# kgnlp/allophant

Measured on AMD Instinct MI355X. Metric: encoder frames/sec (whole node), 10s x 32 utterances @16kHz, higher is better.
Workload: dtype f16x3

## Files before the change

### __graft_entry__.py

```python
import os
import subprocess
import sys

ROOT = os.path.dirname(os.path.abspath(__file__))
if ROOT not in sys.path:
    sys.path.insert(0, ROOT)


def build() -> None:
    jobs = str(min(8, os.cpu_count() or 1))
    subprocess.check_call(["make", "-C", os.path.join(ROOT, "allophant_amd", "csrc"), "-j", jobs])
    out_dir = os.path.join(ROOT, "oracle", "_build")
    os.makedirs(out_dir, exist_ok=True)
    subprocess.check_call(["gcc", "-O2", "-shared", "-fPIC", "-o", os.path.join(out_dir, "liboracle_int.so"),
                           os.path.join(ROOT, "oracle", "oracle_int.c")])
    import allophant_amd
    from allophant_amd import lib

    handle = lib.load()
    missing = [s for s in lib.EXPORTS + lib.ALLOPHONE_EXPORTS + lib.BEAM_EXPORTS + lib.RESAMPLE_EXPORTS + lib.EDIT_EXPORTS + lib.EDIT_WEIGHTED_EXPORTS
               + lib.ALIGN_EXPORTS + lib.SCORE_EXPORTS + lib.SEARCH_EXPORTS + lib.RESTRICT_EXPORTS + lib.LONG_EXPORTS
               if not hasattr(handle, s)]
    if missing:
        raise RuntimeError(f"liballophant_amx.so lacks exported symbols: {missing}")


# ... 45 lines not shown
```

### allophant_amd/csrc/amx_api.hip

```cpp
#include "../../include/allophant_amx.h"
#include "../../include/allophant_amx_allophones.h"
#include "../../include/allophant_amx_beam.h"
#include "../../include/allophant_amx_align.h"
#include "../../include/allophant_amx_score.h"
#include "../../include/allophant_amx_search.h"
#include "../../include/allophant_amx_restrict.h"
#include "../../include/allophant_amx_long.h"
#include "../../include/allophant_amx_resample.h"
#include "../../include/allophant_amx_edit.h"
#include "amx_common.h"

#include <algorithm>
#include <cmath>
#include <cstdio>
#include <cstring>
#include <initializer_list>
#include <map>
#include <cstdlib>
#include <string>
#include <vector>

using namespace amx;

namespace {
// ... 117 lines not shown
    struct GraphEntry {
        std::vector<int64_t> key;
        hipGraphExec_t exec = nullptr;
        hipGraph_t graph = nullptr;
        uint64_t last_use = 0;
        hipStream_t last_stream = nullptr;
    };
    static constexpr int GRAPH_CAP = 32;
    std::vector<GraphEntry> graphs;
    std::vector<std::vector<int64_t>> graph_seen;
    static constexpr int GRAPH_SEEN = 8;
    hipStream_t capture_stream = nullptr;
    bool graph_broken = false;
    uint64_t ws_gen = 0, graph_clock = 0;
    int64_t graph_captures = 0, graph_replays = 0;
    struct RangeSlot {
        int* host = nullptr;
        hipEvent_t ev = nullptr;
        bool pending = false, cont = false;
        uint64_t pass_id = 0;
    };
    static constexpr int RANGE_SLOTS = 8;
    RangeSlot range[RANGE_SLOTS];
    int range_next = 0;
    int64_t range_carry = 0;
    std::string range_carry_ids;
    uint64_t pass_counter = 0;
    int range_chain_seen = 0;
    bool range_chain_open = false;
    int last_N = 0;
// ... 1063 lines not shown
    HIPCHK(h, hipStreamSynchronize(s));
    for (int i = 0; i < amx_handle_s::PIN_SLOTS; ++i) {
        if (h->h_lengths_pinned[i]) {
            (void)hipHostFree(h->h_lengths_pinned[i]);
            (void)hipHostFree(h->h_frames_pinned[i]);
            (void)hipHostFree(h->h_rowoff_pinned[i]);
        }
        HIPCHK(h, hipHostMalloc((void**)&h->h_lengths_pinned[i], (size_t)N * 8));
        HIPCHK(h, hipHostMalloc((void**)&h->h_frames_pinned[i], (size_t)N * 4));
        HIPCHK(h, hipHostMalloc((void**)&h->h_rowoff_pinned[i], (size_t)(3 * N + 1) * 4));
        if (!h->pin_event[i]) HIPCHK(h, hipEventCreateWithFlags(&h->pin_event[i], hipEventDisableTiming));
        h->pin_busy[i] = false;
    }
    h->pinned_cap = N;
    return AMX_OK;
}

static int plan_conv_tiles(amx_handle h, PassPlan& P, int slot, const std::vector<int>& valid_rows, hipStream_t s) {
    const amx_config& c = h->cfg;
    const int N = P.N;
    size_t total_tiles = 0;
    constexpr int64_t TR = GEMM_LN_TILE_ROWS;
    for (int i = 1; i < c.n_conv; ++i) total_tiles += (size_t)((N * P.Ts[i + 1] + TR - 1) / TR);
    if (h->tiles_cap[slot] < total_tiles) {
        if (h->h_tiles_pinned[slot]) (void)hipHostFree(h->h_tiles_pinned[slot]);
        h->h_tiles_pinned[slot] = nullptr;
        h->tiles_cap[slot] = 0;
        HIPCHK(h, hipHostMalloc((void**)&h->h_tiles_pinned[slot], (total_tiles + total_tiles / 4 + 64) * 4));
        h->tiles_cap[slot] = total_tiles + total_tiles / 4 + 64;
    }
// ... 211 lines not shown
        P.frames_host.assign(pin_frames, pin_frames + N);
    }
    P.stream_in_planes = NT == 2;
    if (P.stable && c.layers > 0 && D % 64 == 0 && D <= 2048) {
        WS("ln_rowps", (size_t)P.Mrows * 16, P.ln_rowps);
        WS("ln_coef", (size_t)P.Mrows * 8, P.ln_coef);
        WS("ln_partial", (size_t)P.Mrows * (D / 64) * 8, P.ln_partial);
        const Layer& ly = h->layers[0];
        const int prec = P.prec;
        P.fold = gemm_ln_fold_ok(prec, P.as_consumer(P.qkv_params(h, ly), ly.c_qkv)) &&
                 gemm_ln_fold_ok(prec, P.as_producer(P.oproj_params(h, ly), false)) &&
                 gemm_ln_fold_ok(prec, P.as_consumer(P.ffn1_params(h, ly), ly.c_1)) &&
                 gemm_ln_fold_ok(prec, P.as_producer(P.ffn2_params(h, ly), false)) &&
                 gemm_ln_fold_ok(prec, P.as_producer(P.ffn2_params(h, ly), true));
    }
    ++h->pass_counter;
    h->last_fold = P.fold;
    h->last_packed = P.packed_early ? 2 : (P.packed ? 1 : 0);
    h->last_attention = c.layers > 0 ? attention_form(P.attn_params()) : -1;
    h->last_rows = P.Mrows;
    h->last_graph = 0;
#undef WS
    return AMX_OK;
}

static int enqueue_pass(amx_handle h, const PassPlan& P, hipStream_t s) {
    const amx_config& c = h->cfg;
    const int prec = P.prec, N = P.N, C = P.C, D = P.D, T = P.T;
    const int64_t M = P.M, Mh = P.Mh;
    void* hbuf = P.hbuf;
    bool refused = false;
    auto gemm = [&](const GemmParams& g, int cls = -1) {
        Timed t_(h, cls < 0 ? gemm_class(prec, g) : cls);
        refused |= !launch_gemm(prec, P.with_ws(g), s);
    };
    if (P.needs_qkv_zero) {
        launch_zero(P.qb, P.qkv_bytes, s);
        launch_zero(P.kb, P.qkv_bytes, s);
        launch_zero(P.vtb, P.qkv_bytes, s);
    }
    if (P.packed) {
        const size_t row_b = (size_t)P.dhp * 2, tail = (size_t)(P.TpTot - P.Mp) * row_b, pitch = (size_t)P.TpTot * row_b;
        for (void* buf : {P.qb, P.kb, P.vtb})
            launch_zero_2d((char*)buf + (size_t)P.Mp * row_b, pitch, tail, (size_t)P.NT * P.H, s);
    }
    if (!(P.flags & AMX_FLAG_CONTINUE)) launch_zero(h->nonfinite, 4, s);
    { Timed t_(h, AMX_KC_OTHER); launch_audio_stats(P.d_audio, (const int64_t*)P.d_len, N, P.L, (double*)P.d_partial, (float*)P.d_stats, c.do_normalize, s); }
    if (h->gn) {
        Timed t_(h, AMX_KC_CONV0);
// ... 1243 lines not shown
```

### allophant_amd/csrc/amx_common.h

```cpp
#pragma once
#include <hip/hip_runtime.h>
#include <stdint.h>
#include <string>
#include <type_traits>

struct amx_resample_geometry;
struct amx_resample_row;
struct amx_long_window;
struct amx_long_block;

namespace amx {

typedef _Float16 f16;
typedef __bf16 bf16;
typedef __attribute__((ext_vector_type(8))) _Float16 f16x8;
typedef __attribute__((ext_vector_type(8))) __bf16 bf16x8;
typedef __attribute__((ext_vector_type(4))) _Float16 f16x4;
typedef __attribute__((ext_vector_type(4))) __bf16 bf16x4;
typedef __attribute__((ext_vector_type(2))) _Float16 f16x2;
typedef __attribute__((ext_vector_type(2))) __bf16 bf16x2;
typedef __attribute__((ext_vector_type(2))) float f32x2;
typedef __attribute__((ext_vector_type(4))) float f32x4;
typedef __attribute__((ext_vector_type(16))) float f32x16;

// ... 202 lines not shown
    float* splitk_ws;
    int64_t splitk_ws_elems;
    int splits;
    int64_t split_out;
    const int* tile_list;
    int n_tiles;
    int defer_fixup;
    int a_taps;
    int64_t a_tap_stride;
    unsigned long long* stamps;
    const float4* ln_rowps;
    float2* ln_partial;
    int ln_res_planes;
    const float2* row_coef;
    const float* col_c;
};

extern bool g_force_generic_gemm;
bool launch_gemm(int prec, const GemmParams& p, hipStream_t stream);
bool gemm_uses_pp(int prec, const GemmParams& p);
bool gemm_fuses_ln(int prec, const GemmParams& p);
int gemm_ln_tap_minor_slice(int prec, const GemmParams& p);
int gemm_planned_splits(int prec, const GemmParams& p);
bool fixup_rownorm_eligible(const GemmParams& p);
void launch_fixup_rownorm(int prec, const GemmParams& p, int splits, const float* gamma, const float* beta, float eps, void* out_p,
                          int64_t out_plane, int64_t ldp, float* out_ln, int64_t ldo_ln, hipStream_t stream);
bool gemm_ln_fold_ok(int prec, const GemmParams& p);
void launch_gemm_grouped(int prec, const GemmParams& p, int groups, hipStream_t stream);

struct AttnParams {
    const void* q;
    const void* k;
    const void* v;
    int64_t qk_plane;
    void* out;
    int64_t out_plane;
    const int* frame_len;
    int N, H, T, Tp, dh;
// ... 231 lines not shown
```

### allophant_amd/csrc/amx_gemm.hip

```cpp
#include "amx_common.h"
#include <algorithm>
#include <cstdlib>
#include <type_traits>

namespace amx {

bool g_force_generic_gemm = false;

namespace {

#include "amx_gemm_tile.inc"
#include "amx_gemm_pp.inc"
#include "amx_gemm_ln.inc"

int device_cus() {
    static int per_device[MAX_DEVICES] = {};
    const int dev = current_device();
    int& cus = per_device[dev];
    if (!cus) {
        hipDeviceProp_t prop;
        if (hipGetDeviceProperties(&prop, dev) == hipSuccess) cus = prop.multiProcessorCount;
        if (cus <= 0) cus = 256;
        cus -= cus % 8;
        if (cus < 8) cus = 8;
// ... 125 lines not shown
    q.zbias = q.zoutp = 0;
    return q;
}

template <typename T, int NT, int MI, int NI, int FOLD>
void launch_pp_tiles(const GemmParams& p, int splits, hipStream_t stream) {
    static OncePerDevice attr;
    constexpr int lds = pp::lds_bytes(NT, MI, NI);
    if (attr.first())
        (void)hipFuncSetAttribute((const void*)gemm_pp_kernel<T, NT, MI, NI, FOLD>, hipFuncAttributeMaxDynamicSharedMemorySize, lds);
    if (FOLD) splits = 1;
    const int tiles = ((p.N + NI * 64 - 1) / (NI * 64)) * ((p.M + MI * 32 - 1) / (MI * 32));
    const int cus = device_cus();
    const int units = tiles * splits;
    dim3 grid(units < cus ? units : cus, 1, 1);
    if (splits > 1) {
        hipLaunchKernelGGL((gemm_pp_kernel<T, NT, MI, NI, FOLD>), grid, dim3(512), lds, stream, split_view(p, splits));
        if (!p.defer_fixup) launch_fixup<T, NT>(p, splits, stream);
    } else {
        hipLaunchKernelGGL((gemm_pp_kernel<T, NT, MI, NI, FOLD>), grid, dim3(512), lds, stream, p);
    }
}

void pp_plan(int NT, const GemmParams& p, int* mi_out, int* splits_out, int* ni_out) {
    const int cus = device_cus();
    const double loop = (double)p.K * (NT > 1 ? 3 : 1);
    double best = 1e30;
    *mi_out = 8;
    *splits_out = 1;
    *ni_out = 4;
    for (int mi = 8; mi >= 4; mi -= 4)
        for (int ni = 4; ni >= 3; --ni) {
            const int tiles = ((p.N + ni * 64 - 1) / (ni * 64)) * ((p.M + mi * 32 - 1) / (mi * 32));
            const double per_unit = (480.0 + 60.0 * mi) * (ni == 4 ? 1.0 : 1.1);
            const double unit_loop = loop * mi / 8.0 * (ni == 4 ? 1.0 : 0.75 * 1.06);
            int64_t smax = 1;
// ... 209 lines not shown
    if (p.ln_partial) {
        if (r.ni != 4 || p.N % 64 || p.N > 2048 || !p.out_p || !p.ln_rowps || p.act || p.mode || p.row_len || p.row_coef) return false;
        if (p.ln_res_planes ? NT != 2 : (!p.out_f32 || !p.residual)) return false;
        if (NT == 2 && (p.out_plane != PLANE_IL || p.ldp % 32)) return false;
        if (p.ldp % 8 || ((uintptr_t)p.out_p & 15) || ((uintptr_t)p.ln_partial & 7) || ((uintptr_t)p.ln_rowps & 15)) return false;
    }
    if (p.row_coef) {
        if (!p.col_c || ((uintptr_t)p.col_c & 15) || ((uintptr_t)p.row_coef & 7) || p.residual || p.row_len) return false;
        if (p.mode != 1 && (!p.out_p || p.out_f32)) return false;
    }
    return true;
}

int gemm_planned_splits(int prec, const GemmParams& p) { return route_of(prec, p).splits; }

bool fixup_rownorm_eligible(const GemmParams& p) {
    return p.splitk_ws && p.out_f32 && !p.out_p && p.act == 0 && p.mode == 0 && !p.row_len && !p.ln_gamma && p.N % 4 == 0 &&
           p.N <= 1024 && p.ldo % 4 == 0 && (!p.residual || p.ldr % 4 == 0) && !((uintptr_t)p.out_f32 & 15) &&
           !((uintptr_t)p.residual & 15) && !((uintptr_t)p.bias & 15) && p.zout == 0;
}

void launch_fixup_rownorm(int prec, const GemmParams& p, int splits, const float* gamma, const float* beta, float eps, void* out_p,
                          int64_t out_plane, int64_t ldp, float* out_ln, int64_t ldo_ln, hipStream_t stream) {
    AMX_DISPATCH(prec, (launch_fixup_rownorm_t<T16, NT>(p, splits, gamma, beta, eps, out_p, out_plane, ldp, out_ln, ldo_ln, stream)));
}

bool launch_gemm(int prec, const GemmParams& p_in, hipStream_t stream) {
    const GemmParams p = with_vec_flag(p_in);
    const GemmRoute r = gemm_route(prec_planes(prec), p);
    if (!r.launches) return false;
// ... 11 lines not shown
```

### allophant_amd/csrc/amx_gemm_ln.inc

```

namespace ppw {
constexpr int BM = 128, BN = 512, KS = 32;
static_assert(BM == GEMM_LN_TILE_ROWS, "amx_forward builds the tile lists of ragged batches for this tile height");
constexpr int A_BYTES = BM * 64, W_BYTES = BN * 64, SLOT = A_BYTES + W_BYTES, W_OFF = A_BYTES;
constexpr int LDS_BYTES = 4 * SLOT;
constexpr int EPI_BASE = 2 * SLOT;
constexpr int RED_BASE = EPI_BASE + 8 * pp::EPI_WAVE;
constexpr int AJ = 1, WJ = 4;
}

template <typename T, int NT>
__global__ __launch_bounds__(512, 2) void gemm_ln_kernel(const GemmParams p) {
    typedef typename Vec8<T>::type V8;
    typedef __attribute__((address_space(3))) void* lds_ptr_t;
    extern __shared__ __attribute__((aligned(16))) unsigned char smem[];

    const int tid = threadIdx.x;
    int lane = tid & 63;
    const int wave = __builtin_amdgcn_readfirstlane(tid >> 6);
    const int grp = wave >> 2, wc = wave & 3;
    const int total = p.tile_list ? p.n_tiles : (p.M + ppw::BM - 1) / ppw::BM;

    const int rd_chunk = ((lane >> 4) ^ ((lane >> 2) & 2)) << 4;
    const int a_rd = (grp * 64 + (lane & 15)) * 64 + rd_chunk;
// ... 292 lines not shown
    const int w_rd = ppi::A_BYTES + (grp * 256 + wc * 64 + (lane & 15)) * 128 + rd_chunk;

    const __amdgpu_buffer_rsrc_t w_rsrc = __builtin_amdgcn_make_buffer_rsrc((void*)p.W, 0, -1, 0x00020000);
    uint32_t w_off[2], a_off[4];
#pragma unroll
    for (int par = 0; par < 2; ++par) {
        const int row = (grp * 32 + wc * 8 + par) * 8 + (lane >> 3);
        const int lc = (lane & 7) ^ ((row >> 1) & 7);
        w_off[par] = (uint32_t)((EM * (int64_t)row * p.ldw + lc * 8) * 2);
    }
    const uint32_t w_step = (uint32_t)(p.ldw * 32 * EM);
    int m0 = 0;
    __amdgpu_buffer_rsrc_t a_rsrc;
    auto setup_tile = [&](int i) {
        m0 = (p.tile_list ? p.tile_list[i] : i) * ppi::BM;
        const int64_t b0 = m0 / p.rows_per_batch;
        const int64_t a_tile = b0 * p.a_batch_stride + (m0 - b0 * p.rows_per_batch) * p.lda;
        a_rsrc = __builtin_amdgcn_make_buffer_rsrc((void*)((const T*)p.A + EM * a_tile), 0, -1, 0x00020000);
#pragma unroll
        for (int j = 0; j < 4; ++j) {
            const int row = (wc * 4 + j) * 8 + ((tid & 63) >> 3);
            const int lc = (tid & 7) ^ ((row >> 1) & 7);
            int rr = m0 + row;
            rr = rr < p.M ? rr : p.M - 1;
            const int64_t b = rr / p.rows_per_batch;
            const int64_t t = rr - b * p.rows_per_batch;
            a_off[j] = (uint32_t)((EM * (b * p.a_batch_stride + t * p.lda - a_tile) + lc * 8) * 2);
        }
    };
    const int taps = p.a_taps > 1 ? p.a_taps : 1;
    const uint32_t tap_bytes = (uint32_t)(p.a_tap_stride * EM * 2);
    auto dma_slice = [&](int slot, int slice) {
        unsigned char* base = smem + slot * ppi::SLICE;
        const uint32_t so = (uint32_t)slice * 128;
        if (grp == 0) {
            uint32_t so_a = so;
            if (taps > 1) {
                const uint32_t cs = (uint32_t)slice / (uint32_t)taps, pos = (uint32_t)slice - cs * (uint32_t)taps;
                const uint32_t tap = pos ? (uint32_t)taps - pos : 0u;
                so_a = tap * tap_bytes + cs * 128;
            }
#pragma unroll
// ... 28 lines not shown
#pragma unroll
        for (int prod = 0; prod < NT + 1; ++prod) {
            const int pw = NT == 2 ? (prod == 1 ? 1 : 0) : prod, pa = NT == 2 ? (prod == 2 ? 1 : 0) : prod;
#pragma unroll
            for (int ni = 0; ni < 4; ++ni)
#pragma unroll
                for (int mi = 0; mi < MI; ++mi) mfma16_acc(acc[ni][mi], fw[pw][ni], fa[pa][mi]);
        }
        __builtin_amdgcn_s_setprio(0);
        asm volatile("s_waitcnt vmcnt(0)" ::: "memory");
        __builtin_amdgcn_sched_barrier(0);
        __builtin_amdgcn_s_barrier();
        __builtin_amdgcn_sched_barrier(0);
    };

    int it = blockIdx.x;
    setup_tile(it);
    dma_slice(0, 0);
    for (;;) {
#pragma unroll
        for (int i = 0; i < 4; ++i)
#pragma unroll
            for (int j = 0; j < MI; ++j) acc[i][j] = f32x4{0.f, 0.f, 0.f, 0.f};
        const int nk = p.K / KSL;
        asm volatile("s_waitcnt vmcnt(0)" ::: "memory");
        __builtin_amdgcn_s_barrier();
        if (grp == 1) __builtin_amdgcn_s_barrier();
        for (int k = 0; k < nk; k += 2) {
            phase(std::integral_constant<int, 0>{}, k, nk);
            phase(std::integral_constant<int, 1>{}, k + 1, nk);
        }
        if (grp == 0) __builtin_amdgcn_s_barrier();
        asm volatile("s_nop 15\n\ts_nop 15" ::: "memory");

        const int mw = m0, nw = grp * 256 + wc * 64;
        const int next = it + gridDim.x;
        const bool has_next = next < total;
        if (has_next) {
            setup_tile(next);
            dma_slice(0, 0);
        }

        asm volatile("" : "+v"(lane));
        {
            const int lr = lane & 15, lg = lane >> 4;
            const float scale = p.scale;
            float* red = (float*)(smem + ppi::RED_BASE);
#pragma unroll
            for (int ni = 0; ni < 4; ++ni) {
                const float4 b4 = p.bias ? *(const float4*)(p.bias + nw + ni * 16 + 4 * lg) : make_float4(0.f, 0.f, 0.f, 0.f);
#pragma unroll
                for (int mi = 0; mi < MI; ++mi) {
                    acc[ni][mi][0] = fmaf(acc[ni][mi][0], scale, b4.x);
                    acc[ni][mi][1] = fmaf(acc[ni][mi][1], scale, b4.y);
                    acc[ni][mi][2] = fmaf(acc[ni][mi][2], scale, b4.z);
                    acc[ni][mi][3] = fmaf(acc[ni][mi][3], scale, b4.w);
// ... 43 lines not shown
                for (int mi = 0; mi < MI; ++mi) {
                    const f32x2 g01 = gelu_fast2(f32x2{fmaf((acc[ni][mi][0] - mean[mi]) * rstd[mi], g4.x, e4.x),
                                                       fmaf((acc[ni][mi][1] - mean[mi]) * rstd[mi], g4.y, e4.y)});
                    const f32x2 g23 = gelu_fast2(f32x2{fmaf((acc[ni][mi][2] - mean[mi]) * rstd[mi], g4.z, e4.z),
                                                       fmaf((acc[ni][mi][3] - mean[mi]) * rstd[mi], g4.w, e4.w)});
                    acc[ni][mi][0] = g01[0];
                    acc[ni][mi][1] = g01[1];
                    acc[ni][mi][2] = g23[0];
                    acc[ni][mi][3] = g23[1];
                }
            }
            float* es = (float*)(smem + ppi::EPI_BASE + wave * pp::EPI_WAVE);
            if (mw + ppi::BM <= p.M) pp_epilogue_p16<T, NT, false, false, MI, true>(p, acc, es, lane, mw, nw);
            else pp_epilogue_generic<T, NT, MI, true>(p, acc, es, lane, mw, nw, nullptr);
        }
        if (!has_next) break;
        it = next;
        lgkm_wait0();
        __builtin_amdgcn_s_barrier();
    }
}
```

### allophant_amd/csrc/amx_gemm_pp.inc

```

namespace pp {
constexpr int BN = 256;
constexpr int EPI_WAVE = 32 * 64 * 4;
template <int MI, int NI = 4>
struct Ring {
    static constexpr int A_BYTES = MI * 32 * 128, W_BYTES = NI * 64 * 128, SLICE = A_BYTES + W_BYTES;
    static constexpr int NSL = MI == 8 ? 2 : 3, DIST = NSL - 1;
    static constexpr int EPI_BASE = DIST * SLICE;
    static constexpr int LDS_BYTES = (NSL * SLICE > EPI_BASE + 8 * EPI_WAVE) ? NSL * SLICE : EPI_BASE + 8 * EPI_WAVE;
};
constexpr int lds_bytes(int NT, int MI, int NI = 4) {
    return MI == 8 ? (NI == 4 ? Ring<8, 4>::LDS_BYTES : Ring<8, 3>::LDS_BYTES) : (NI == 4 ? Ring<4, 4>::LDS_BYTES : Ring<4, 3>::LDS_BYTES);
}
constexpr int epi_base(int NT, int MI, int NI = 4) {
    return MI == 8 ? (NI == 4 ? Ring<8, 4>::EPI_BASE : Ring<8, 3>::EPI_BASE) : (NI == 4 ? Ring<4, 4>::EPI_BASE : Ring<4, 3>::EPI_BASE);
}
__device__ __forceinline__ int es_idx(int row, int chunk) { return row * 64 + ((chunk ^ (row & 7)) << 2); }
}

__device__ __forceinline__ void mfma16_acc(f32x4& c, f16x8 a, f16x8 b) {
    asm volatile("v_mfma_f32_16x16x32_f16 %0, %1, %2, %0" : "+v"(c) : "v"(a), "v"(b));
}
__device__ __forceinline__ void mfma16_acc(f32x4& c, bf16x8 a, bf16x8 b) {
    asm volatile("v_mfma_f32_16x16x32_bf16 %0, %1, %2, %0" : "+v"(c) : "v"(a), "v"(b));
// ... 204 lines not shown
    for (int q = 0; q < MI / 2; ++q) {
        float2 cf[4];
        if (COEF) {
#pragma unroll
            for (int i = 0; i < 4; ++i) cf[i] = cf_all[q][i];
        }
        pp_stage_round(es, acc, q, lane);
        f32x4 c[4][2];
#pragma unroll
        for (int i = 0; i < 4; ++i) {
            c[i][0] = *(const f32x4*)(es + pp::es_idx(i * 8 + rs, 2 * c8));
            c[i][1] = *(const f32x4*)(es + pp::es_idx(i * 8 + rs, 2 * c8 + 1));
        }
#pragma unroll
        for (int i = 0; i < 4; ++i) {
            float v[8];
            if (COEF) {
                const float as = cf[i].x * scale, bs = cf[i].y;
                v[0] = fmaf(c[i][0][0], as, fmaf(bs, cc0.x, b0.x)); v[1] = fmaf(c[i][0][1], as, fmaf(bs, cc0.y, b0.y));
                v[2] = fmaf(c[i][0][2], as, fmaf(bs, cc0.z, b0.z)); v[3] = fmaf(c[i][0][3], as, fmaf(bs, cc0.w, b0.w));
                v[4] = fmaf(c[i][1][0], as, fmaf(bs, cc1.x, b1.x)); v[5] = fmaf(c[i][1][1], as, fmaf(bs, cc1.y, b1.y));
                v[6] = fmaf(c[i][1][2], as, fmaf(bs, cc1.z, b1.z)); v[7] = fmaf(c[i][1][3], as, fmaf(bs, cc1.w, b1.w));
            } else {
                v[0] = fmaf(c[i][0][0], scale, b0.x); v[1] = fmaf(c[i][0][1], scale, b0.y); v[2] = fmaf(c[i][0][2], scale, b0.z);
                v[3] = fmaf(c[i][0][3], scale, b0.w); v[4] = fmaf(c[i][1][0], scale, b1.x); v[5] = fmaf(c[i][1][1], scale, b1.y);
                v[6] = fmaf(c[i][1][2], scale, b1.z); v[7] = fmaf(c[i][1][3], scale, b1.w);
            }
            union { typename Vec2<T>::type h[4]; V8 v; } hv, lv;
#pragma unroll
            for (int r = 0; r < 4; ++r) {
                f32x2 x = {v[2 * r], v[2 * r + 1]};
                if (ACT) x = gelu_fast2(x);
                lv.h[r] = typename Vec2<T>::type{(T)0.f, (T)0.f};
                split16x2<T, NT>(x, hv.h[r], lv.h[r]);
            }
            T* dst;
            if (QK) {
                dst = base + ((int64_t)b * p.H * p.Tp + t) * row_stride;
                t += 8;
                const bool wrap = t >= p.T;
                t -= wrap ? p.T : 0;
                b += wrap ? 1 : 0;
            } else {
                dst = base + (int64_t)(q * 32 + i * 8) * row_stride;
            }
            *(V8*)dst = hv.v;
// ... 137 lines not shown
    int lane = tid & 63;
    const int wave = __builtin_amdgcn_readfirstlane(tid >> 6);
    const int grp = wave >> 2, wc = wave & 3;
    const int ntn = (p.N + BNK - 1) / BNK, ntm = (p.M + BMK - 1) / BMK;
    const int tiles = ntn * ntm;
    const int total = tiles * p.splits;

    const int rd_chunk = ((lane >> 4) ^ ((lane >> 1) & 7)) << 4;
    const int a_rd = (grp * HALF + (lane & 15)) * 128 + rd_chunk;
    const int w_rd = R::A_BYTES + (wc * (16 * NI) + (lane & 15)) * 128 + rd_chunk;

    int m0 = 0, n0 = 0, ks = 0;
    __amdgpu_buffer_rsrc_t a_rsrc, w_rsrc;
    uint32_t a_off[4], w_off[2];
    const uint32_t w_step = (uint32_t)(p.ldw * 32 * EM);
    auto setup_tile = [&](int unit) {
        ks = unit / tiles;
        const int i = unit - ks * tiles;
        const int total = tiles;
        const int xcd = i & 7, q = total >> 3, r = total & 7;
        const int j = (xcd < r ? xcd * (q + 1) : r * (q + 1) + (xcd - r) * q) + (i >> 3);
        constexpr int GM = 8;
        const int per_group = GM * ntn;
        const int group = j / per_group;
        const int first_m = group * GM;
        const int gsize = ntm - first_m < GM ? ntm - first_m : GM;
        const int in_group = j - group * per_group;
        m0 = (first_m + in_group % gsize) * BMK;
        n0 = (in_group / gsize) * BNK;
        const int m0c = m0 < p.M ? m0 : p.M - 1, n0c = n0 < p.N ? n0 : p.N - 1;
        const int64_t b0 = m0c / p.rows_per_batch;
        const int64_t a_tile = b0 * p.a_batch_stride + (m0c - b0 * p.rows_per_batch) * p.lda;
        const int64_t k_first = (int64_t)ks * p.K;
        a_rsrc = __builtin_amdgcn_make_buffer_rsrc((void*)((const T*)p.A + EM * (a_tile + k_first)), 0, -1, 0x00020000);
        const int64_t w_bytes = ((int64_t)(p.N - n0c) * p.ldw - k_first) * 2 * EM;
        w_rsrc = __builtin_amdgcn_make_buffer_rsrc((void*)((const T*)p.W + EM * ((int64_t)n0c * p.ldw + k_first)), 0,
                                                   (int)(uint32_t)(w_bytes < 0xFFFFFFFFll ? w_bytes : 0xFFFFFFFFll), 0x00020000);
#pragma unroll
        for (int jj = 0; jj < APW2; ++jj) {
            const int row = (grp * (2 * MI) + wc * APW2 + jj) * 8 + ((tid & 63) >> 3);
            const int lc = (tid & 7) ^ ((row >> 1) & 7);
            int rr = m0 + row;
            rr = rr < p.M ? rr : p.M - 1;
            const int64_t b = rr / p.rows_per_batch;
            const int64_t t = rr - b * p.rows_per_batch;
            a_off[jj] = (uint32_t)((EM * (b * p.a_batch_stride + t * p.lda - a_tile) + lc * 8) * 2);
        }
#pragma unroll
        for (int par = 0; par < 2; ++par) {
            const int row = (wc * WPW + par) * 8 + ((tid & 63) >> 3);
            const int lc = (tid & 7) ^ ((row >> 1) & 7);
            w_off[par] = (uint32_t)((EM * (int64_t)row * p.ldw + lc * 8) * 2);
        }
    };

    f32x4 acc[NI][MI];
    V8 fa[2][MI], fw[2][NI];

    auto dma_slice = [&](int slot, int slice) {
#ifdef AMX_ABLATE_NO_DMA
        return;
#endif
        unsigned char* base = smem + slot * R::SLICE;
        const uint32_t so = (uint32_t)slice * 128;
#pragma unroll
        for (int j = 0; j < APW2; ++j)
            __builtin_amdgcn_raw_ptr_buffer_load_lds(a_rsrc, (lds_ptr_t)(base + (grp * (2 * MI) + wc * APW2 + j) * 1024), 16, a_off[j], so,
// ... 16 lines not shown
            case 1: asm volatile("s_waitcnt vmcnt(1)" ::: "memory"); break;
            case 2: asm volatile("s_waitcnt vmcnt(2)" ::: "memory"); break;
            case 3: asm volatile("s_waitcnt vmcnt(3)" ::: "memory"); break;
            case 4: asm volatile("s_waitcnt vmcnt(4)" ::: "memory"); break;
            case 5: asm volatile("s_waitcnt vmcnt(5)" ::: "memory"); break;
            case 6: asm volatile("s_waitcnt vmcnt(6)" ::: "memory"); break;
            case 7: asm volatile("s_waitcnt vmcnt(7)" ::: "memory"); break;
            case 8: asm volatile("s_waitcnt vmcnt(8)" ::: "memory"); break;
            case 9: asm volatile("s_waitcnt vmcnt(9)" ::: "memory"); break;
            case 10: asm volatile("s_waitcnt vmcnt(10)" ::: "memory"); break;
            case 11: asm volatile("s_waitcnt vmcnt(11)" ::: "memory"); break;
            default: asm volatile("s_waitcnt vmcnt(12)" ::: "memory"); break;
        }
    };
#ifdef AMX_PP_STAMP
    unsigned long long st_load = 0, st_bar1 = 0, st_mfma = 0, st_vm = 0, st_bar2 = 0, st_prev = 0, st_begin_rt = 0, st_loop = 0;
    auto stamp = []() -> unsigned long long {
        unsigned long long t;
        __builtin_amdgcn_sched_barrier(0);
        asm volatile("s_memtime %0\n\ts_waitcnt lgkmcnt(0)" : "=s"(t)::"memory");
        __builtin_amdgcn_sched_barrier(0);
        return t;
    };
    {
        unsigned long long t;
        asm volatile("s_memrealtime %0\n\ts_waitcnt lgkmcnt(0)" : "=s"(t)::"memory");
        st_begin_rt = t;
    }
    const unsigned long long st_begin = stamp();
#endif
    auto phase = [&](auto slot_c, int k, int nk) {
// ... 45 lines not shown
        const unsigned long long t3 = stamp();
        st_mfma += t3 - t2;
#endif
        if (R::DIST == 2 && k + 2 < nk) wait_dma(grp == 0 ? CNT_A + CNT_W : CNT_A);
        else asm volatile("s_waitcnt vmcnt(0)" ::: "memory");
#ifdef AMX_PP_STAMP
        const unsigned long long t4 = stamp();
        st_vm += t4 - t3;
        st_prev = t4;
#endif
        __builtin_amdgcn_sched_barrier(0);
        __builtin_amdgcn_s_barrier();
        __builtin_amdgcn_sched_barrier(0);
    };
    int it = blockIdx.x;
    setup_tile(it);
    stage_head();
    for (;;) {
#pragma unroll
        for (int i = 0; i < NI; ++i)
#pragma unroll
            for (int j = 0; j < MI; ++j) acc[i][j] = f32x4{0.f, 0.f, 0.f, 0.f};
#ifdef AMX_PP_STAMP
        const unsigned long long st_l0 = stamp();
        st_prev = 0;
#endif
        {
            const int nk = p.K / KSL;
            if (R::DIST == 2) wait_dma(grp == 0 ? APW2 + WPW : APW2);
            else asm volatile("s_waitcnt vmcnt(0)" ::: "memory");
            __builtin_amdgcn_s_barrier();
// ... 2 lines not shown
                for (int k = 0; k < nk; k += 2) {
                    phase(std::integral_constant<int, 0>{}, k, nk);
                    phase(std::integral_constant<int, 1>{}, k + 1, nk);
                }
            } else {
                for (int k = 0;;) {
                    phase(std::integral_constant<int, 0>{}, k, nk);
                    if (++k == nk) break;
                    phase(std::integral_constant<int, 1>{}, k, nk);
                    if (++k == nk) break;
                    phase(std::integral_constant<int, 2>{}, k, nk);
                    if (++k == nk) break;
                }
            }
        }
        if (grp == 0) __builtin_amdgcn_s_barrier();
        asm volatile("s_nop 15\n\ts_nop 15" ::: "memory");
#ifdef AMX_PP_STAMP
        st_loop += stamp() - st_l0;
#endif

        const int mw = m0 + grp * HALF, nw = n0 + wc * (16 * NI);
        float* out_f32 = p.out_f32 ? p.out_f32 + (int64_t)ks * p.split_out : nullptr;
        const int next = it + gridDim.x;
        const bool has_next = next < total;
        if (has_next) {
            setup_tile(next);
            stage_head();
        }

#ifndef AMX_ABLATE_NO_EPI
        asm volatile("" : "+v"(lane));
        if (nw < p.N && mw < p.M) {
            float* es = (float*)(smem + pp::epi_base(NT, MI, NI) + wave * pp::EPI_WAVE);
            bool done = false;
            if constexpr (FOLD == 1) {
                if (mw + HALF <= p.M && nw + 16 * NI <= p.N && p.vec_ok) {
                    if (p.mode == 1) {
                        if (p.T >= 8 && p.dh % 8 == 0 && p.qk_plane % 8 == 0 && !(((uintptr_t)p.q | (uintptr_t)p.k | (uintptr_t)p.v) & 15)) {
                            pp_epilogue_p16<T, NT, false, true, MI, false, NI, true>(p, acc, es, lane, mw, nw);
                            done = true;
                        }
                    } else if (p.out_p && !p.out_f32 && p.ldp % 8 == 0 && p.out_plane % 8 == 0 && !((uintptr_t)p.out_p & 15)) {
                        if (p.act == 1) pp_epilogue_p16<T, NT, true, false, MI, false, NI, true>(p, acc, es, lane, mw, nw);
// ... 31 lines not shown
                } else if (p.out_p && !p.out_f32 && !p.residual && p.ldp % 8 == 0 && p.out_plane % 8 == 0 && !((uintptr_t)p.out_p & 15)) {
                    if (p.act == 1) pp_epilogue_p16<T, NT, true, false, MI, false, NI>(p, acc, es, lane, mw, nw);
                    else pp_epilogue_p16<T, NT, false, false, MI, false, NI>(p, acc, es, lane, mw, nw);
                    done = true;
                }
            }
            if (!done) pp_epilogue_generic<T, NT, MI, false, NI>(p, acc, es, lane, mw, nw, out_f32);
            }
        }
#else
#pragma unroll
        for (int i = 0; i < NI; ++i)
#pragma unroll
            for (int j = 0; j < MI; ++j) asm volatile("" ::"v"(acc[i][j]));
#endif
        if (!has_next) break;
        it = next;
        lgkm_wait0();
        __builtin_amdgcn_s_barrier();
    }
#ifdef AMX_PP_STAMP
    if (p.stamps && (wave == 0 || wave == 4) && (tid & 63) == 0) {
        const unsigned long long st_end = stamp();
        unsigned long long rt;
        asm volatile("s_memrealtime %0\n\ts_waitcnt lgkmcnt(0)" : "=s"(rt)::"memory");
        unsigned long long* o = p.stamps + ((int64_t)blockIdx.x * 2 + (wave >> 2)) * 10;
        o[0] = st_load; o[1] = st_bar1; o[2] = st_mfma; o[3] = st_vm; o[4] = st_bar2; o[5] = st_loop;
        o[6] = rt - st_begin_rt; o[7] = 1; o[8] = st_end - st_begin; o[9] = (unsigned long long)((total - (int)blockIdx.x + (int)gridDim.x - 1) / (int)gridDim.x);
    }
#endif
}
```

Before: 543,400.

## Precompute GEMM tile walk tables and simplify per-tile address setup

Adds host-built device tables mapping each persistent-GEMM work unit to its (m, n, k-split) tile, so the kernel reads them through the constant address space instead of doing integer divisions per tile. Row-offset setup switches to 32-bit arithmetic, with a fast path for single-batch inputs and a bounded subtract loop in place of 64-bit divides. The next tile's entry is fetched before the barrier, the COEF epilogue is vectorized into packed fma, and extra timing stamps are added. The risks are an extra table allocation and lookup on the first pass, since tables are only built before the next pass; the subtract loop also assumes a tile spans at most two batch boundaries.

```diff
diff --git a/__graft_entry__.py b/__graft_entry__.py
--- a/__graft_entry__.py
+++ b/__graft_entry__.py
@@ -9,7 +9,7 @@
 
 def build() -> None:
     jobs = str(min(8, os.cpu_count() or 1))
-    subprocess.check_call(["make", "-C", os.path.join(ROOT, "allophant_amd", "csrc"), "-j", jobs])
+    subprocess.check_call(["make", "-C", os.path.join(ROOT, "allophant_amd", "csrc"), "-j", jobs, "all", "check-programs"])
     out_dir = os.path.join(ROOT, "oracle", "_build")
     os.makedirs(out_dir, exist_ok=True)
     subprocess.check_call(["gcc", "-O2", "-shared", "-fPIC", "-o", os.path.join(out_dir, "liboracle_int.so"),
diff --git a/allophant_amd/csrc/amx_api.hip b/allophant_amd/csrc/amx_api.hip
--- a/allophant_amd/csrc/amx_api.hip
+++ b/allophant_amd/csrc/amx_api.hip
@@ -155,6 +155,8 @@
     bool graph_broken = false;
     uint64_t ws_gen = 0, graph_clock = 0;
     int64_t graph_captures = 0, graph_replays = 0;
+    std::map<unsigned long long, const unsigned long long*> tile_tables;
+    std::vector<unsigned long long> tile_tables_wanted;
     struct RangeSlot {
         int* host = nullptr;
         hipEvent_t ev = nullptr;
@@ -1248,6 +1250,31 @@
     }
     h->pinned_cap = N;
     return AMX_OK;
+}
+
+static int plan_tile_tables(amx_handle h) {
+    for (const unsigned long long key : h->tile_tables_wanted) {
+        if (h->tile_tables.count(key)) continue;
+        const std::vector<uint64_t> walk = pp_tile_table((int)(uint32_t)key, (int)((key >> 32) & 0xFFFFFF), (int)(key >> 56));
+        void* d = dev_alloc(h, walk.size() * 8, false);
+        if (!d) return fail(h, AMX_ENOMEM, "tile walk table allocation failed");
+        HIPCHK(h, hipMemcpy(d, walk.data(), walk.size() * 8, hipMemcpyHostToDevice));
+        h->tile_tables[key] = (const unsigned long long*)d;
+    }
+    h->tile_tables_wanted.clear();
+    return AMX_OK;
+}
+
+static void attach_tile_table(amx_handle h, int prec, GemmParams& g) {
+    const unsigned long long key = gemm_pp_tile_table_key(prec, g);
+    if (!key) return;
+    const auto it = h->tile_tables.find(key);
+    if (it != h->tile_tables.end()) {
+        g.tile_table = it->second;
+        g.tile_table_key = key;
+    } else if (std::find(h->tile_tables_wanted.begin(), h->tile_tables_wanted.end(), key) == h->tile_tables_wanted.end()) {
+        h->tile_tables_wanted.push_back(key);
+    }
 }
 
 static int plan_conv_tiles(amx_handle h, PassPlan& P, int slot, const std::vector<int>& valid_rows, hipStream_t s) {
@@ -1489,6 +1516,7 @@
                  gemm_ln_fold_ok(prec, P.as_producer(P.ffn2_params(h, ly), false)) &&
                  gemm_ln_fold_ok(prec, P.as_producer(P.ffn2_params(h, ly), true));
     }
+    if ((rc = plan_tile_tables(h))) return rc;
     ++h->pass_counter;
     h->last_fold = P.fold;
     h->last_packed = P.packed_early ? 2 : (P.packed ? 1 : 0);
@@ -1507,7 +1535,9 @@
     bool refused = false;
     auto gemm = [&](const GemmParams& g, int cls = -1) {
         Timed t_(h, cls < 0 ? gemm_class(prec, g) : cls);
-        refused |= !launch_gemm(prec, P.with_ws(g), s);
+        GemmParams q = P.with_ws(g);
+        attach_tile_table(h, prec, q);
+        refused |= !launch_gemm(prec, q, s);
     };
     if (P.needs_qkv_zero) {
         launch_zero(P.qb, P.qkv_bytes, s);
diff --git a/allophant_amd/csrc/amx_common.h b/allophant_amd/csrc/amx_common.h
--- a/allophant_amd/csrc/amx_common.h
+++ b/allophant_amd/csrc/amx_common.h
@@ -1,5 +1,6 @@
 #pragma once
 #include <hip/hip_runtime.h>
+#include "amx_gemm_walk.h"
 #include <stdint.h>
 #include <string>
 #include <type_traits>
@@ -240,6 +241,8 @@
     int ln_res_planes;
     const float2* row_coef;
     const float* col_c;
+    const unsigned long long* tile_table;
+    unsigned long long tile_table_key;
 };
 
 extern bool g_force_generic_gemm;
@@ -248,6 +251,7 @@
 bool gemm_fuses_ln(int prec, const GemmParams& p);
 int gemm_ln_tap_minor_slice(int prec, const GemmParams& p);
 int gemm_planned_splits(int prec, const GemmParams& p);
+unsigned long long gemm_pp_tile_table_key(int prec, const GemmParams& p);
 bool fixup_rownorm_eligible(const GemmParams& p);
 void launch_fixup_rownorm(int prec, const GemmParams& p, int splits, const float* gamma, const float* beta, float eps, void* out_p,
                           int64_t out_plane, int64_t ldp, float* out_ln, int64_t ldo_ln, hipStream_t stream);
diff --git a/allophant_amd/csrc/amx_gemm.hip b/allophant_amd/csrc/amx_gemm.hip
--- a/allophant_amd/csrc/amx_gemm.hip
+++ b/allophant_amd/csrc/amx_gemm.hip
@@ -163,12 +163,10 @@
     const int cus = device_cus();
     const int units = tiles * splits;
     dim3 grid(units < cus ? units : cus, 1, 1);
-    if (splits > 1) {
-        hipLaunchKernelGGL((gemm_pp_kernel<T, NT, MI, NI, FOLD>), grid, dim3(512), lds, stream, split_view(p, splits));
-        if (!p.defer_fixup) launch_fixup<T, NT>(p, splits, stream);
-    } else {
-        hipLaunchKernelGGL((gemm_pp_kernel<T, NT, MI, NI, FOLD>), grid, dim3(512), lds, stream, p);
-    }
+    GemmParams q = splits > 1 ? split_view(p, splits) : p;
+    if (q.tile_table_key != pp_tile_table_key((p.M + MI * 32 - 1) / (MI * 32), (p.N + NI * 64 - 1) / (NI * 64), splits)) q.tile_table = nullptr;
+    hipLaunchKernelGGL((gemm_pp_kernel<T, NT, MI, NI, FOLD>), grid, dim3(512), lds, stream, q);
+    if (splits > 1 && !p.defer_fixup) launch_fixup<T, NT>(p, splits, stream);
 }
 
 void pp_plan(int NT, const GemmParams& p, int* mi_out, int* splits_out, int* ni_out) {
@@ -408,6 +406,14 @@
 
 int gemm_planned_splits(int prec, const GemmParams& p) { return route_of(prec, p).splits; }
 
+unsigned long long gemm_pp_tile_table_key(int prec, const GemmParams& p) {
+    const GemmRoute r = route_of(prec, p);
+    if (r.kernel != GemmKernel::PP || !r.launches || r.fold == 2) return 0;
+    const int ntm = (p.M + r.mi * 32 - 1) / (r.mi * 32), ntn = (p.N + r.ni * 64 - 1) / (r.ni * 64);
+    const int splits = r.fold ? 1 : r.splits;
+    return pp_tile_table_ok(ntm, ntn, splits) ? pp_tile_table_key(ntm, ntn, splits) : 0;
+}
+
 bool fixup_rownorm_eligible(const GemmParams& p) {
     return p.splitk_ws && p.out_f32 && !p.out_p && p.act == 0 && p.mode == 0 && !p.row_len && !p.ln_gamma && p.N % 4 == 0 &&
            p.N <= 1024 && p.ldo % 4 == 0 && (!p.residual || p.ldr % 4 == 0) && !((uintptr_t)p.out_f32 & 15) &&
diff --git a/allophant_amd/csrc/amx_gemm_ln.inc b/allophant_amd/csrc/amx_gemm_ln.inc
--- a/allophant_amd/csrc/amx_gemm_ln.inc
+++ b/allophant_amd/csrc/amx_gemm_ln.inc
@@ -330,18 +330,34 @@
     __amdgpu_buffer_rsrc_t a_rsrc;
     auto setup_tile = [&](int i) {
         m0 = (p.tile_list ? p.tile_list[i] : i) * ppi::BM;
-        const int64_t b0 = m0 / p.rows_per_batch;
-        const int64_t a_tile = b0 * p.a_batch_stride + (m0 - b0 * p.rows_per_batch) * p.lda;
+        const bool one_batch = p.rows_per_batch >= (int64_t)p.M;
+        uint32_t b0 = 0, t0 = (uint32_t)m0;
+        const uint32_t rpb = (uint32_t)p.rows_per_batch;
+        if (!one_batch) {
+            b0 = (uint32_t)m0 / rpb;
+            t0 = (uint32_t)m0 - b0 * rpb;
+        }
+        const int64_t a_tile = (int64_t)b0 * p.a_batch_stride + (int64_t)t0 * p.lda;
         a_rsrc = __builtin_amdgcn_make_buffer_rsrc((void*)((const T*)p.A + EM * a_tile), 0, -1, 0x00020000);
+        const uint32_t lda_b = (uint32_t)p.lda * (2 * EM), batch_b = (uint32_t)p.a_batch_stride * (2 * EM);
+        const int last = p.M - 1 - m0;
 #pragma unroll
         for (int j = 0; j < 4; ++j) {
             const int row = (wc * 4 + j) * 8 + ((tid & 63) >> 3);
             const int lc = (tid & 7) ^ ((row >> 1) & 7);
-            int rr = m0 + row;
-            rr = rr < p.M ? rr : p.M - 1;
-            const int64_t b = rr / p.rows_per_batch;
-            const int64_t t = rr - b * p.rows_per_batch;
-            a_off[j] = (uint32_t)((EM * (b * p.a_batch_stride + t * p.lda - a_tile) + lc * 8) * 2);
+            const uint32_t d = (uint32_t)(row < last ? row : last);
+            if (one_batch) {
+                a_off[j] = d * lda_b + (uint32_t)lc * 16;
+            } else {
+                uint32_t t = t0 + d, db = 0;
+#pragma unroll
+                for (int c = 0; c < 2; ++c) {
+                    const bool over = t >= rpb;
+                    t -= over ? rpb : 0;
+                    db += over ? 1 : 0;
+                }
+                a_off[j] = db * batch_b + (t - t0) * lda_b + (uint32_t)lc * 16;
+            }
         }
     };
     const int taps = p.a_taps > 1 ? p.a_taps : 1;
@@ -400,10 +416,25 @@
         __builtin_amdgcn_sched_barrier(0);
     };
 
+#ifdef AMX_PP_STAMP
+    unsigned long long st_loop = 0, st_setup = 0, st_epi = 0, st_begin_rt = 0;
+    auto stamp = []() -> unsigned long long {
+        unsigned long long t;
+        __builtin_amdgcn_sched_barrier(0);
+        asm volatile("s_memtime %0\n\ts_waitcnt lgkmcnt(0)" : "=s"(t)::"memory");
+        __builtin_amdgcn_sched_barrier(0);
+        return t;
+    };
+    asm volatile("s_memrealtime %0\n\ts_waitcnt lgkmcnt(0)" : "=s"(st_begin_rt)::"memory");
+    const unsigned long long st_begin = stamp();
+#endif
     int it = blockIdx.x;
     setup_tile(it);
     dma_slice(0, 0);
     for (;;) {
+#ifdef AMX_PP_STAMP
+        const unsigned long long st_l0 = stamp();
+#endif
 #pragma unroll
         for (int i = 0; i < 4; ++i)
 #pragma unroll
@@ -422,10 +453,18 @@
         const int mw = m0, nw = grp * 256 + wc * 64;
         const int next = it + gridDim.x;
         const bool has_next = next < total;
+#ifdef AMX_PP_STAMP
+        const unsigned long long st_s0 = stamp();
+        st_loop += st_s0 - st_l0;
+#endif
         if (has_next) {
             setup_tile(next);
             dma_slice(0, 0);
         }
+#ifdef AMX_PP_STAMP
+        const unsigned long long st_s1 = stamp();
+        st_setup += st_s1 - st_s0;
+#endif
 
         asm volatile("" : "+v"(lane));
         {
@@ -499,9 +538,23 @@
             if (mw + ppi::BM <= p.M) pp_epilogue_p16<T, NT, false, false, MI, true>(p, acc, es, lane, mw, nw);
             else pp_epilogue_generic<T, NT, MI, true>(p, acc, es, lane, mw, nw, nullptr);
         }
+#ifdef AMX_PP_STAMP
+        st_epi += stamp() - st_s1;
+#endif
         if (!has_next) break;
         it = next;
         lgkm_wait0();
         __builtin_amdgcn_s_barrier();
     }
+#ifdef AMX_PP_STAMP
+    if (p.stamps && (wave == 0 || wave == 4) && (tid & 63) == 0) {
+        const unsigned long long st_end = stamp();
+        unsigned long long rt;
+        asm volatile("s_memrealtime %0\n\ts_waitcnt lgkmcnt(0)" : "=s"(rt)::"memory");
+        unsigned long long* o = p.stamps + ((int64_t)blockIdx.x * 2 + (wave >> 2)) * 12;
+        o[0] = o[1] = o[2] = o[3] = o[4] = 0; o[5] = st_loop;
+        o[6] = rt - st_begin_rt; o[7] = 1; o[8] = st_end - st_begin; o[9] = (unsigned long long)((total - (int)blockIdx.x + (int)gridDim.x - 1) / (int)gridDim.x);
+        o[10] = st_setup; o[11] = st_epi;
+    }
+#endif
 }
diff --git a/allophant_amd/csrc/amx_gemm_pp.inc b/allophant_amd/csrc/amx_gemm_pp.inc
--- a/allophant_amd/csrc/amx_gemm_pp.inc
+++ b/allophant_amd/csrc/amx_gemm_pp.inc
@@ -242,22 +242,28 @@
         }
 #pragma unroll
         for (int i = 0; i < 4; ++i) {
-            float v[8];
+            f32x2 v2[4];
             if (COEF) {
                 const float as = cf[i].x * scale, bs = cf[i].y;
-                v[0] = fmaf(c[i][0][0], as, fmaf(bs, cc0.x, b0.x)); v[1] = fmaf(c[i][0][1], as, fmaf(bs, cc0.y, b0.y));
-                v[2] = fmaf(c[i][0][2], as, fmaf(bs, cc0.z, b0.z)); v[3] = fmaf(c[i][0][3], as, fmaf(bs, cc0.w, b0.w));
-                v[4] = fmaf(c[i][1][0], as, fmaf(bs, cc1.x, b1.x)); v[5] = fmaf(c[i][1][1], as, fmaf(bs, cc1.y, b1.y));
-                v[6] = fmaf(c[i][1][2], as, fmaf(bs, cc1.z, b1.z)); v[7] = fmaf(c[i][1][3], as, fmaf(bs, cc1.w, b1.w));
+                const f32x2 as2 = {as, as}, bs2 = {bs, bs};
+                v2[0] = __builtin_elementwise_fma(__builtin_shufflevector(c[i][0], c[i][0], 0, 1), as2,
+                                                  __builtin_elementwise_fma(bs2, f32x2{cc0.x, cc0.y}, f32x2{b0.x, b0.y}));
+                v2[1] = __builtin_elementwise_fma(__builtin_shufflevector(c[i][0], c[i][0], 2, 3), as2,
+                                                  __builtin_elementwise_fma(bs2, f32x2{cc0.z, cc0.w}, f32x2{b0.z, b0.w}));
+                v2[2] = __builtin_elementwise_fma(__builtin_shufflevector(c[i][1], c[i][1], 0, 1), as2,
+                                                  __builtin_elementwise_fma(bs2, f32x2{cc1.x, cc1.y}, f32x2{b1.x, b1.y}));
+                v2[3] = __builtin_elementwise_fma(__builtin_shufflevector(c[i][1], c[i][1], 2, 3), as2,
+                                                  __builtin_elementwise_fma(bs2, f32x2{cc1.z, cc1.w}, f32x2{b1.z, b1.w}));
             } else {
-                v[0] = fmaf(c[i][0][0], scale, b0.x); v[1] = fmaf(c[i][0][1], scale, b0.y); v[2] = fmaf(c[i][0][2], scale, b0.z);
-                v[3] = fmaf(c[i][0][3], scale, b0.w); v[4] = fmaf(c[i][1][0], scale, b1.x); v[5] = fmaf(c[i][1][1], scale, b1.y);
-                v[6] = fmaf(c[i][1][2], scale, b1.z); v[7] = fmaf(c[i][1][3], scale, b1.w);
+                v2[0] = f32x2{fmaf(c[i][0][0], scale, b0.x), fmaf(c[i][0][1], scale, b0.y)};
+                v2[1] = f32x2{fmaf(c[i][0][2], scale, b0.z), fmaf(c[i][0][3], scale, b0.w)};
+                v2[2] = f32x2{fmaf(c[i][1][0], scale, b1.x), fmaf(c[i][1][1], scale, b1.y)};
+                v2[3] = f32x2{fmaf(c[i][1][2], scale, b1.z), fmaf(c[i][1][3], scale, b1.w)};
             }
             union { typename Vec2<T>::type h[4]; V8 v; } hv, lv;
 #pragma unroll
             for (int r = 0; r < 4; ++r) {
-                f32x2 x = {v[2 * r], v[2 * r + 1]};
+                f32x2 x = v2[r];
                 if (ACT) x = gelu_fast2(x);
                 lv.h[r] = typename Vec2<T>::type{(T)0.f, (T)0.f};
                 split16x2<T, NT>(x, hv.h[r], lv.h[r]);
@@ -425,43 +431,87 @@
     __amdgpu_buffer_rsrc_t a_rsrc, w_rsrc;
     uint32_t a_off[4], w_off[2];
     const uint32_t w_step = (uint32_t)(p.ldw * 32 * EM);
-    auto setup_tile = [&](int unit) {
-        ks = unit / tiles;
-        const int i = unit - ks * tiles;
-        const int total = tiles;
-        const int xcd = i & 7, q = total >> 3, r = total & 7;
-        const int j = (xcd < r ? xcd * (q + 1) : r * (q + 1) + (xcd - r) * q) + (i >> 3);
-        constexpr int GM = 8;
-        const int per_group = GM * ntn;
-        const int group = j / per_group;
-        const int first_m = group * GM;
-        const int gsize = ntm - first_m < GM ? ntm - first_m : GM;
-        const int in_group = j - group * per_group;
-        m0 = (first_m + in_group % gsize) * BMK;
-        n0 = (in_group / gsize) * BNK;
+    constexpr bool TABLED = FOLD != 2;
+    if constexpr (TABLED) {
+#pragma unroll
+        for (int par = 0; par < 2; ++par) {
+            const int row = (wc * WPW + par) * 8 + ((tid & 63) >> 3);
+            const int lc = (tid & 7) ^ ((row >> 1) & 7);
+            w_off[par] = (uint32_t)((EM * (int64_t)row * p.ldw + lc * 8) * 2);
+        }
+    }
+    typedef const __attribute__((address_space(4))) unsigned long long* walk_ptr_t;
+    auto walk_entry = [&](int unit) -> unsigned long long {
+        if constexpr (TABLED) {
+            const walk_ptr_t table = (walk_ptr_t)(uintptr_t)p.tile_table;
+            if (table) return table[unit];
+        }
+        return pp_walk_unit(unit, ntm, ntn);
+    };
+    auto setup_tile = [&](unsigned long long entry) {
+        m0 = (int)(uint32_t)entry * BMK;
+        n0 = (int)((uint32_t)(entry >> 32) & 0xFFFFFFu) * BNK;
+        ks = (int)(entry >> 56);
         const int m0c = m0 < p.M ? m0 : p.M - 1, n0c = n0 < p.N ? n0 : p.N - 1;
-        const int64_t b0 = m0c / p.rows_per_batch;
-        const int64_t a_tile = b0 * p.a_batch_stride + (m0c - b0 * p.rows_per_batch) * p.lda;
+        const bool one_batch = p.rows_per_batch >= (int64_t)p.M;
+        uint32_t b0 = 0, t0 = (uint32_t)m0c;
+        const uint32_t rpb = (uint32_t)p.rows_per_batch;
+        int64_t a_tile;
+        if constexpr (TABLED) {
+            if (!one_batch) {
+                b0 = (uint32_t)m0c / rpb;
+                t0 = (uint32_t)m0c - b0 * rpb;
+            }
+            a_tile = (int64_t)b0 * p.a_batch_stride + (int64_t)t0 * p.lda;
+        } else {
+            const int64_t b0l = m0c / p.rows_per_batch;
+            a_tile = b0l * p.a_batch_stride + (m0c - b0l * p.rows_per_batch) * p.lda;
+        }
         const int64_t k_first = (int64_t)ks * p.K;
         a_rsrc = __builtin_amdgcn_make_buffer_rsrc((void*)((const T*)p.A + EM * (a_tile + k_first)), 0, -1, 0x00020000);
         const int64_t w_bytes = ((int64_t)(p.N - n0c) * p.ldw - k_first) * 2 * EM;
         w_rsrc = __builtin_amdgcn_make_buffer_rsrc((void*)((const T*)p.W + EM * ((int64_t)n0c * p.ldw + k_first)), 0,
                                                    (int)(uint32_t)(w_bytes < 0xFFFFFFFFll ? w_bytes : 0xFFFFFFFFll), 0x00020000);
-#pragma unroll
-        for (int jj = 0; jj < APW2; ++jj) {
-            const int row = (grp * (2 * MI) + wc * APW2 + jj) * 8 + ((tid & 63) >> 3);
-            const int lc = (tid & 7) ^ ((row >> 1) & 7);
-            int rr = m0 + row;
-            rr = rr < p.M ? rr : p.M - 1;
-            const int64_t b = rr / p.rows_per_batch;
-            const int64_t t = rr - b * p.rows_per_batch;
-            a_off[jj] = (uint32_t)((EM * (b * p.a_batch_stride + t * p.lda - a_tile) + lc * 8) * 2);
-        }
-#pragma unroll
-        for (int par = 0; par < 2; ++par) {
-            const int row = (wc * WPW + par) * 8 + ((tid & 63) >> 3);
-            const int lc = (tid & 7) ^ ((row >> 1) & 7);
-            w_off[par] = (uint32_t)((EM * (int64_t)row * p.ldw + lc * 8) * 2);
+        if constexpr (TABLED) {
+            const uint32_t lda_b = (uint32_t)p.lda * (2 * EM), batch_b = (uint32_t)p.a_batch_stride * (2 * EM);
+            const int last = p.M - 1 - m0c;
+            int ln = tid & 63;
+            asm volatile("" : "+v"(ln));
+#pragma unroll
+            for (int jj = 0; jj < APW2; ++jj) {
+                const int row = (grp * (2 * MI) + wc * APW2 + jj) * 8 + (ln >> 3);
+                const int lc = (ln & 7) ^ ((row >> 1) & 7);
+                const uint32_t d = (uint32_t)(row < last ? row : last);
+                if (one_batch) {
+                    a_off[jj] = d * lda_b + (uint32_t)lc * 16;
+                } else {
+                    uint32_t t = t0 + d, db = 0;
+#pragma unroll
+                    for (int c = 0; c < 2; ++c) {
+                        const bool over = t >= rpb;
+                        t -= over ? rpb : 0;
+                        db += over ? 1 : 0;
+                    }
+                    a_off[jj] = db * batch_b + (t - t0) * lda_b + (uint32_t)lc * 16;
+                }
+            }
+        } else {
+#pragma unroll
+            for (int jj = 0; jj < APW2; ++jj) {
+                const int row = (grp * (2 * MI) + wc * APW2 + jj) * 8 + ((tid & 63) >> 3);
+                const int lc = (tid & 7) ^ ((row >> 1) & 7);
+                int rr = m0 + row;
+                rr = rr < p.M ? rr : p.M - 1;
+                const int64_t b = rr / p.rows_per_batch;
+                const int64_t t = rr - b * p.rows_per_batch;
+                a_off[jj] = (uint32_t)((EM * (b * p.a_batch_stride + t * p.lda - a_tile) + lc * 8) * 2);
+            }
+#pragma unroll
+            for (int par = 0; par < 2; ++par) {
+                const int row = (wc * WPW + par) * 8 + ((tid & 63) >> 3);
+                const int lc = (tid & 7) ^ ((row >> 1) & 7);
+                w_off[par] = (uint32_t)((EM * (int64_t)row * p.ldw + lc * 8) * 2);
+            }
         }
     };
 
@@ -508,7 +558,8 @@
         }
     };
 #ifdef AMX_PP_STAMP
-    unsigned long long st_load = 0, st_bar1 = 0, st_mfma = 0, st_vm = 0, st_bar2 = 0, st_prev = 0, st_begin_rt = 0, st_loop = 0;
+    unsigned long long st_load = 0, st_bar1 = 0, st_mfma = 0, st_vm = 0, st_bar2 = 0, st_prev = 0, st_begin_rt = 0, st_loop = 0,
+                       st_setup = 0, st_epi = 0;
     auto stamp = []() -> unsigned long long {
         unsigned long long t;
         __builtin_amdgcn_sched_barrier(0);
@@ -584,7 +635,7 @@
         __builtin_amdgcn_sched_barrier(0);
     };
     int it = blockIdx.x;
-    setup_tile(it);
+    setup_tile(walk_entry(it));
     stage_head();
     for (;;) {
 #pragma unroll
@@ -617,20 +668,30 @@
                 }
             }
         }
+        const int next = it + gridDim.x;
+        const bool has_next = next < total;
+        unsigned long long next_entry = 0;
+        if (TABLED && has_next) next_entry = walk_entry(next);
         if (grp == 0) __builtin_amdgcn_s_barrier();
         asm volatile("s_nop 15\n\ts_nop 15" ::: "memory");
+        if (!TABLED && has_next) next_entry = walk_entry(next);
 #ifdef AMX_PP_STAMP
         st_loop += stamp() - st_l0;
 #endif
 
         const int mw = m0 + grp * HALF, nw = n0 + wc * (16 * NI);
         float* out_f32 = p.out_f32 ? p.out_f32 + (int64_t)ks * p.split_out : nullptr;
-        const int next = it + gridDim.x;
-        const bool has_next = next < total;
+#ifdef AMX_PP_STAMP
+        const unsigned long long st_s0 = stamp();
+#endif
         if (has_next) {
-            setup_tile(next);
+            setup_tile(next_entry);
             stage_head();
         }
+#ifdef AMX_PP_STAMP
+        const unsigned long long st_s1 = stamp();
+        st_setup += st_s1 - st_s0;
+#endif
 
 #ifndef AMX_ABLATE_NO_EPI
         asm volatile("" : "+v"(lane));
@@ -692,6 +753,9 @@
 #pragma unroll
             for (int j = 0; j < MI; ++j) asm volatile("" ::"v"(acc[i][j]));
 #endif
+#ifdef AMX_PP_STAMP
+        st_epi += stamp() - st_s1;
+#endif
         if (!has_next) break;
         it = next;
         lgkm_wait0();
@@ -702,9 +766,10 @@
         const unsigned long long st_end = stamp();
         unsigned long long rt;
         asm volatile("s_memrealtime %0\n\ts_waitcnt lgkmcnt(0)" : "=s"(rt)::"memory");
-        unsigned long long* o = p.stamps + ((int64_t)blockIdx.x * 2 + (wave >> 2)) * 10;
+        unsigned long long* o = p.stamps + ((int64_t)blockIdx.x * 2 + (wave >> 2)) * 12;
         o[0] = st_load; o[1] = st_bar1; o[2] = st_mfma; o[3] = st_vm; o[4] = st_bar2; o[5] = st_loop;
         o[6] = rt - st_begin_rt; o[7] = 1; o[8] = st_end - st_begin; o[9] = (unsigned long long)((total - (int)blockIdx.x + (int)gridDim.x - 1) / (int)gridDim.x);
-    }
-#endif
-}
+        o[10] = st_setup; o[11] = st_epi;
+    }
+#endif
+}
diff --git a/allophant_amd/csrc/amx_gemm_walk.h b/allophant_amd/csrc/amx_gemm_walk.h
--- /dev/null
+++ b/allophant_amd/csrc/amx_gemm_walk.h
@@ -0,0 +1,44 @@
+#pragma once
+#include <cstddef>
+#include <cstdint>
+#include <vector>
+
+#if defined(__HIPCC__) || defined(__CUDACC__)
+#define AMX_WALK_FN __host__ __device__ inline
+#else
+#define AMX_WALK_FN inline
+#endif
+
+namespace amx {
+
+constexpr int PP_WALK_MAX_TN = 1 << 24, PP_WALK_MAX_KS = 1 << 8;
+AMX_WALK_FN uint64_t pp_walk_pack(uint32_t tm, uint32_t tn, uint32_t ks) { return (uint64_t)tm | ((uint64_t)tn << 32) | ((uint64_t)ks << 56); }
+
+AMX_WALK_FN uint64_t pp_walk_unit(int unit, int ntm, int ntn) {
+    const int tiles = ntm * ntn;
+    const int ks = unit / tiles;
+    const int i = unit - ks * tiles;
+    const int xcd = i & 7, q = tiles >> 3, r = tiles & 7;
+    const int j = (xcd < r ? xcd * (q + 1) : r * (q + 1) + (xcd - r) * q) + (i >> 3);
+    constexpr int GM = 8;
+    const int per_group = GM * ntn;
+    const int group = j / per_group;
+    const int first_m = group * GM;
+    const int gsize = ntm - first_m < GM ? ntm - first_m : GM;
+    const int in_group = j - group * per_group;
+    return pp_walk_pack((uint32_t)(first_m + in_group % gsize), (uint32_t)(in_group / gsize), (uint32_t)ks);
+}
+
+constexpr int64_t PP_WALK_MAX_UNITS = 1 << 16;
+inline bool pp_tile_table_ok(int ntm, int ntn, int splits) {
+    return ntm > 0 && ntn > 0 && splits > 0 && ntn < PP_WALK_MAX_TN && splits < PP_WALK_MAX_KS &&
+           (int64_t)ntm * ntn * splits <= PP_WALK_MAX_UNITS;
+}
+inline uint64_t pp_tile_table_key(int ntm, int ntn, int splits) { return pp_walk_pack((uint32_t)ntm, (uint32_t)ntn, (uint32_t)splits); }
+inline std::vector<uint64_t> pp_tile_table(int ntm, int ntn, int splits) {
+    std::vector<uint64_t> t((size_t)ntm * ntn * splits);
+    for (size_t u = 0; u < t.size(); ++u) t[u] = pp_walk_unit((int)u, ntm, ntn);
+    return t;
+}
+
+}
```

After: 542,800. No clear change (-0.1%).
